# lcicek/Critic-VAE

Measured on AMD Instinct MI355X. Metric: VAE train-step images/sec on 64x64x3 frames, higher is better.
Workload: dtype f32

## Files before the change

### critic-vae_amd/csrc/common.h

```cpp
#pragma once
#include <hip/hip_runtime.h>
#include <stdint.h>
#include <stddef.h>
#include <atomic>

typedef float f32x16 __attribute__((ext_vector_type(16)));
typedef float f32x4 __attribute__((ext_vector_type(4)));
typedef __bf16 bf16x8 __attribute__((ext_vector_type(8)));

typedef __bf16 bf16x4 __attribute__((ext_vector_type(4)));

template <typename AT> struct Act;
template <> struct Act<float> {
    static constexpr bool BF16 = false;
    static __device__ __forceinline__ float ld(const float* p, size_t i) { return p[i]; }
    static __device__ __forceinline__ void st(float* p, size_t i, float v) { p[i] = v; }
    static __device__ __forceinline__ f32x4 ld4(const float* p, size_t i) { return *reinterpret_cast<const f32x4*>(p + i); }
    static __device__ __forceinline__ void st4(float* p, size_t i, f32x4 v) { *reinterpret_cast<f32x4*>(p + i) = v; }
    template <int V> using Vec = float __attribute__((ext_vector_type(V)));
    template <int V> static __device__ __forceinline__ Vec<V> ldv(const float* p, size_t i) {
        static_assert(V == 1 || V == 4, "fp32 storage: scalar or float4 accesses");
        return *reinterpret_cast<const Vec<V>*>(p + i);
    }
    template <int V> static __device__ __forceinline__ void stv(float* p, size_t i, Vec<V> v) {
// ... 63 lines not shown
    static constexpr int TILES_PER_IMG = tile_geom(H).TILES_PER_IMG;
    static_assert(TW * TH * IMGS == 128, "tile must hold 128 pixels");
};

__host__ __device__ inline int cdiv(int a, int b) { return (a + b - 1) / b; }

__device__ __forceinline__ void vm_drained() { __builtin_amdgcn_s_waitcnt(0x0F70); }

__device__ __forceinline__ int xcd_tile(int x, int G) { return (G & 7) ? x : (x & 7) * (G >> 3) + (x >> 3); }
inline int64_t align_up(int64_t v, int64_t a) { return (v + a - 1) / a * a; }

__device__ __forceinline__ float wave_sum(float v) {
#pragma unroll
    for (int o = 32; o > 0; o >>= 1) v += __shfl_xor(v, o, 64);
    return v;
}
__device__ __forceinline__ double wave_sum_d(double v) {
#pragma unroll
    for (int o = 32; o > 0; o >>= 1) v += __shfl_xor(v, o, 64);
    return v;
}

__device__ __forceinline__ bool wg_arrive_last(unsigned* counter, unsigned total, unsigned* lds_word) {
    asm volatile("s_waitcnt vmcnt(0)" ::: "memory");
    __syncthreads();
    if (threadIdx.x == 0) {
        __builtin_amdgcn_fence(__ATOMIC_RELEASE, "agent");
        asm volatile("s_waitcnt vmcnt(0)" ::: "memory");
        const unsigned t = __hip_atomic_fetch_add(counter, 1u, __ATOMIC_RELAXED, __HIP_MEMORY_SCOPE_AGENT);
        const bool last = t == total - 1;
        if (last) {
            __hip_atomic_store(counter, 0u, __ATOMIC_RELAXED, __HIP_MEMORY_SCOPE_AGENT);
            __builtin_amdgcn_fence(__ATOMIC_ACQUIRE, "agent");
            asm volatile("s_waitcnt vmcnt(0)" ::: "memory");
        }
        *lds_word = last ? 1u : 0u;
    }
    __syncthreads();
    return *lds_word != 0u;
}

void cvae_probe_begin(hipStream_t st);
void cvae_probe_end(hipStream_t st);

void cvae_set_error(const char* fmt, ...);
#define CVAE_CHECK_LAUNCH()                                                        \
    do {                                                                           \
        hipError_t e_ = hipGetLastError();                                         \
        if (e_ != hipSuccess) {                                                    \
            cvae_set_error("%s:%d launch failed: %s", __FILE__, __LINE__,          \
                           hipGetErrorString(e_));                                 \
            return (int)e_;                                                        \
        }                                                                          \
    } while (0)

struct DeviceOnce { std::atomic<uint64_t> mask{0}; };
inline int cvae_grant_lds(DeviceOnce& once, const void* kernel, int bytes) {
    int dev = 0;
    hipError_t e = hipGetDevice(&dev);
    const uint64_t bit = 1ull << (dev & 63);
    if (e == hipSuccess && (once.mask.load(std::memory_order_acquire) & bit)) return 0;
    if (e == hipSuccess) e = hipFuncSetAttribute(kernel, hipFuncAttributeMaxDynamicSharedMemorySize, bytes);
    if (e != hipSuccess) { cvae_set_error("dynamic LDS opt-in (%d bytes) failed: %s", bytes, hipGetErrorString(e)); return (int)e; }
    once.mask.fetch_or(bit, std::memory_order_release);
    return 0;
}

int cvae_num_cus();
int persistent_grid(int wgs_per_cu, int num_items);

enum ConvFamily { CONV_PER_TILE = 0, CONV_PS = 1, CONV_BIG = 2, E1_PACKED_FRAME = 1 };
struct ConvRoute {
    ConvFamily family;
    int tilesPerPartial;
};
ConvRoute conv_route(int precision, int layer, int width, bool dgrad, int64_t B);

int launch_conv_fwd(int layer, int width, int B, const float* in, const float* w, const float* bias,
                    float* out, float* bnpart, float* ws, hipStream_t st);
int64_t conv_fwd_ws_floats(int layer, int width, int B);
int launch_conv_dgrad(int layer, int width, int B, const float* dout, const float* w,
                      const float* mask_src, float* din, float* ws, hipStream_t st);
int64_t conv_dgrad_ws_floats(int layer, int width, int B);
bool conv_bf16_supported(int layer, int width);
int64_t conv_bf16_pack_floats(int ns);
int launch_pack_w_bf16(const float* const w[4], float* packed, int ns, hipStream_t st);
int launch_conv_fwd_bf16(int layer, int width, int ns, int B, const float* in, const float* packed, const float* bias, float* out,
                         float* bnpart, float* ws, hipStream_t st, int* tilesPerPartial = nullptr);
int launch_conv_dgrad_bf16(int layer, int width, int ns, int B, const float* dout, const float* packed, float* din, float* ws, hipStream_t st);
int launch_pack_up_bf16(const float* const wc[3], float* packed, int ns, hipStream_t st);
int launch_conv_up_fwd_bf16(int layer, int width, int ns, int B, const float* in, const float* packed, const float* bias, float* out, hipStream_t st);
int launch_conv_up_dgrad_bf16(int layer, int width, int ns, int B, const float* dout, const float* packed, const float* aux, float* din, hipStream_t st);
int64_t wgrad_bf16_ws_floats(int layer, int width, int B);
int launch_conv_wgrad_bf16(int layer, int width, int B, const float* in, const float* dout, float* dw, float* dbias, float* ws, hipStream_t st);
bool conv_wgrad_split_supported(int products);
int64_t wgrad_split_ws_floats(int layer, int width, int B);
int launch_conv_wgrad_split(int layer, int width, int products, int B, const float* in, const float* dout, float* dw, float* dbias,
                            float* ws, hipStream_t st);
int launch_splitk_bias_relu(const float* slab, const float* bias, float* out, int64_t slice, int KS, int C, hipStream_t st, bool out_bf16 = false);
int64_t wgrad_ws_floats(int layer, int width, int B);
int launch_conv_wgrad(int layer, int width, int B, const float* in, const float* dout, float* dw,
                      float* dbias, float* ws, hipStream_t st);
int launch_reduce_slabs(const float* slab, float* dst, int64_t n, int S, int64_t stride, hipStream_t st,
                        float* mid = nullptr, bool out_bf16 = false);
int launch_colsum(const float* src, int64_t rows, int C, float* dst, float* ws, hipStream_t st);
int64_t colsum_ws_floats(int64_t rows, int C);
static constexpr int CS_BLOCKS = 128;
__device__ __forceinline__ void colsum_stage1_block(const float* __restrict__ src, int64_t rows, int C, float* __restrict__ part,
                                                    int blk, int nblk, float* red) {
    const int c = threadIdx.x % C, rl = threadIdx.x / C, RL = 256 / C;
    const int64_t per = (rows + nblk - 1) / nblk;
    const int64_t r0 = blk * per;
    int64_t r1 = r0 + per; if (r1 > rows) r1 = rows;
    float acc = 0.f;
    for (int64_t r = r0 + rl; r < r1; r += RL) acc += src[r * C + c];
    red[threadIdx.x] = acc;
    __syncthreads();
    if (rl == 0) {
        for (int k = 1; k < RL; ++k) acc += red[k * C + c];
        part[(size_t)blk * C + c] = acc;
    }
}
int64_t col_reduce_ws_floats(int W);
int launch_col_reduce_partial(const float* in, int R, int W, int64_t stride, float* ws, hipStream_t st,
                              const float** rows_out, int* R_out, int64_t* stride_out);
int launch_col_reduce(const float* in, int R, int W, int64_t stride, float* out, float* ws, hipStream_t st, int skip_col0 = -1);
int launch_e1_fwd(int width, int B, const float* x, const float* w, const float* bias, float* y,
                  float* bnpart, hipStream_t st, bool bf16 = false, int pass = 0, const float* coef = nullptr, float* a1 = nullptr,
                  float* xp = nullptr);
int launch_e1_wgrad(int width, int B, const float* x, const float* dy, float* dw, float* dbias, float* ws,
                    hipStream_t st, bool bf16 = false, const float* const* fuse = nullptr,
                    const float* xp = nullptr);
const float* bn_bwd_bcoef(int layer, int width, int B, const float* ws);
int64_t e1_wgrad_ws_floats(int width, int B);
int launch_d4_fwd(int width, int B, const float* in, const float* w, const float* bias, float* recon,
                  hipStream_t st, bool bf16io = false);
int64_t d4_bwd_ws_floats(int width, int B);
int launch_d4_bwd(int width, int B, const float* o3, const float* d_recon, const float* recon,
                  const float* w, float* dout, float* d_o3, float* dw, float* db, float* ws,
                  hipStream_t st, bool bf16io = false);
int64_t conv_up_wc_floats(int layer);
int launch_collapse_w(int layer, const float* w, float* wc, hipStream_t st);
int launch_collapse_w3(const float* const w[3], float* const wc[3], hipStream_t st);
int64_t conv_up_ws_floats(int layer, int width, int B);
int launch_conv_up_fwd(int layer, int width, int B, const float* in, const float* wc, const float* bias,
                       float* out, float* ws, hipStream_t st);
int launch_conv_up_dgrad(int layer, int width, int B, const float* dout, const float* wc, const float* aux,
                         float* din, float* ws, hipStream_t st);
int64_t conv_up_wgrad_ws_floats(int layer, int width, int B);
int launch_conv_up_wgrad(int layer, int width, int B, const float* in, const float* dout, float* dw,
                         float* dbias, float* ws, hipStream_t st, bool bf16 = false);
int launch_up_wgrad_bf16_main(int layer, int width, int B, const float* in, const float* dout, float* slab, int Smax, int* S_out, hipStream_t st,
                              int* plan = nullptr);
int conv_wgrad_bf16_plan(int layer, int width, int B, int plan[3]);
int conv_up_wgrad_bf16_plan(int layer, int width, int B, int plan[3]);
int bn_num_tiles(int layer, int width, int B);
int launch_bn_fwd_finalize(int layer, int width, int B, const float* bnpart, const float* gamma,
                           const float* beta, float* run_mean, float* run_var, float* coef,
                           float* ws, int train, hipStream_t st, int tilesPerPartial = 1);
int launch_bn_fwd_record(int layer, int width, int B, const float* bnpart, float* ws, hipStream_t st, int tilesPerPartial,
                         double* rec, double* count);
int launch_bn_fwd_finish(int layer, int width, const double* rec, const double* count, const float* gamma, const float* beta,
                         float* run_mean, float* run_var, float* coef, hipStream_t st);
int64_t bn_fwd_ws_floats(int layer, int width);
int launch_bn_pool_act_fwd(int layer, int width, int B, const float* y, const float* coef, float* a,
                           hipStream_t st, bool bf16io = false);
// ... 119 lines not shown
```

### critic-vae_amd/csrc/conv_mfma_ps.hip

```cpp
#include "common.h"
#include "conv_epilogue.h"

struct ConvPsArgs {
    const float* in;
    const float* w;
    const float* bias;
    float* out;
    float* bnpart;
    int B;
};

typedef unsigned u32x4p __attribute__((ext_vector_type(4)));
__device__ __forceinline__ __amdgpu_buffer_rsrc_t make_rsrc_f(const void* p, unsigned bytes) {
    return __builtin_amdgcn_make_buffer_rsrc(const_cast<void*>(p), 0, (int)bytes, 0x00020000);
}
static constexpr unsigned OOBF = 0x80000000u;

template <int NT> struct KChunkPs { static constexpr int KC = NT == 32 ? 32 : 16, KCP = KC + 1; };

template <int KCH, int NCH, int H, bool DGRAD, int NT, int EPI>
__global__ __launch_bounds__(256) __attribute__((amdgpu_waves_per_eu(2, 2))) void conv5x5_mfma_ps_kernel(ConvPsArgs a, int numTiles) {
    using T = Tile<H>;
    constexpr int NB = NT / 32, NY = NCH / NT;
    constexpr int KC = KChunkPs<NT>::KC, KCP = KChunkPs<NT>::KCP, QPP = KC / 4, NCHUNK = KCH / KC;
// ... 154 lines not shown
                }
            }
    };

    if constexpr (HAS_BIAS) { for (int c = tid; c < NCH; c += 256) lds_bias[c] = a.bias[c]; }
    Item cur = setup(tile, n0), pd = cur;
    bool have_pd = false;
    load_w(cur, 0, 0);
    load_input(cur, 0);
    __syncthreads();
    int itemNo = 0;
    for (;;) {
        if (((itemNo++ ^ (blockIdx.x >= (unsigned)(G / 2))) & 1) != 0) __builtin_amdgcn_s_setprio(1); else __builtin_amdgcn_s_setprio(0);
        int itn = it + G, tilen, n0n;
        decode(itn, tilen, n0n);
        const bool have_next = itn < numItems && tilen < numTiles;
        const Item nxt = have_next ? setup(tilen, n0n) : cur;
#pragma unroll
        for (int nb = 0; nb < NB; ++nb)
#pragma unroll
            for (int g = 0; g < 4; ++g) {
                const f32x4 b4 = HAS_BIAS ? *reinterpret_cast<const f32x4*>(lds_bias + cur.n0 + nb * 32 + 8 * g + 4 * lh) : f32x4{0.f, 0.f, 0.f, 0.f};
#pragma unroll
                for (int e = 0; e < 4; ++e) acc[nb][4 * g + e] = b4[e];
            }
#pragma unroll
        for (int r = 0; r < 5; ++r) {
            __syncthreads();
            if (r == 0) store_input();
            store_w();
            if (r == 0) { if (NCHUNK > 1) load_input(cur, 1); else load_input(nxt, 0); }
            if (r < 4) load_w(cur, 0, r + 1); else if (NCHUNK > 1) load_w(cur, 1, 0); else load_w(nxt, 0, 0);
            __builtin_amdgcn_sched_barrier(0);
            if (r == 0) drain_store(pd, have_pd, 0, 0);
            if (r == 1) { drain_store(pd, have_pd, 0, 2); bn_rows(pd, 0); }
            if (r == 2 && NB > 1) { drain_store(pd, have_pd, NB - 1, 0); bn_rows(pd, NB - 1); }
            if (r == 3 && NB > 1) drain_store(pd, have_pd, NB - 1, 2);
            if (r == 4) bn_combine(pd, have_pd);
            __syncthreads();
            mfma_phase(r);
        }
        for (int cc = 1; cc < NCHUNK; ++cc) {
            const bool lastc = cc == NCHUNK - 1;
#pragma unroll
            for (int r = 0; r < 5; ++r) {
                __syncthreads();
                if (r == 0) store_input();
                store_w();
                if (r == 0) { if (lastc) load_input(nxt, 0); else load_input(cur, cc + 1); }
                if (r < 4) load_w(cur, cc, r + 1); else if (lastc) load_w(nxt, 0, 0); else load_w(cur, cc + 1, 0);
                __syncthreads();
                mfma_phase(r);
            }
        }
#pragma unroll
        for (int nb = 0; nb < NB; ++nb)
#pragma unroll
            for (int v = 0; v < 16; ++v) pend[nb][v] = RELU ? fmaxf(acc[nb][v], 0.f) : acc[nb][v];
        pd = cur; have_pd = true;
        if (!have_next) break;
        cur = nxt; it = itn;
    }
#pragma unroll
    for (int nb = 0; nb < NB; ++nb) { drain_store(pd, true, nb, 0); drain_store(pd, true, nb, 2); bn_rows(pd, nb); }
    __syncthreads();
    bn_combine(pd, true);
}

template <int KCH, int NCH, int H, bool DGRAD, int NT, int EPI>
static int run_mfma_ps(const ConvPsArgs& a, hipStream_t st) {
    using T = Tile<H>;
    constexpr int NY = NCH / NT;
    const int numTiles = cdiv(a.B, T::IMGS) * T::TILES_PER_IMG;
    const int G = persistent_grid(2, cdiv(numTiles, 8) * 8 * NY);
    cvae_probe_begin(st);
    hipLaunchKernelGGL((conv5x5_mfma_ps_kernel<KCH, NCH, H, DGRAD, NT, EPI>), dim3(G), dim3(256), 0, st, a, numTiles);
    cvae_probe_end(st);
    CVAE_CHECK_LAUNCH();
    return 0;
}

int launch_conv_mfma_ps(int layer, int width, bool dgrad, int B, const float* in, const float* w, const float* bias, float* out, float* bnpart, hipStream_t st) {
    const ConvPsArgs a{in, w, bias, out, bnpart, B};
    if (!dgrad) {
        if (width == 64) {
            switch (layer) {
                case 1: return run_mfma_ps<32, 64, 32, false, 64, EPI_BIAS_BNSTAT>(a, st);
                case 2: return run_mfma_ps<64, 128, 16, false, 64, EPI_BIAS_BNSTAT>(a, st);
                case 3: return run_mfma_ps<128, 256, 8, false, 64, EPI_BIAS_BNSTAT>(a, st);
            }
        } else if (width == 128) {
            switch (layer) {
                case 1: return run_mfma_ps<32, 64, 64, false, 64, EPI_BIAS_BNSTAT>(a, st);
                case 2: return run_mfma_ps<64, 128, 32, false, 64, EPI_BIAS_BNSTAT>(a, st);
            }
        }
    } else {
        if (width == 64) {
            switch (layer) {
                case 2: return run_mfma_ps<128, 64, 16, true, 64, EPI_PLAIN>(a, st);
                case 3: return run_mfma_ps<256, 128, 8, true, 64, EPI_PLAIN>(a, st);
            }
        } else if (width == 128) {
            switch (layer) {
                case 2: return run_mfma_ps<128, 64, 32, true, 64, EPI_PLAIN>(a, st);
            }
        }
    }
    cvae_set_error("conv_mfma_ps: no instantiation for layer %d %s at width %d", layer, dgrad ? "dgrad" : "fwd", width);
    return -2;
}
```

### critic-vae_amd/lib.py

```python
import ctypes as C
import os
import subprocess

import torch

_HERE = os.path.dirname(os.path.abspath(__file__))
LIB_PATH = os.environ.get("CVAE_LIB") or os.path.join(_HERE, "libcvae_hip.so")
N_SCALARS = 16
SYNC_DOUBLES = 2412
SYNC_POINTS = 9
SCORE_COLS = 8
SCORE_STATE_DOUBLES = 24


class CvaeError(RuntimeError):
    pass


class _Config(C.Structure):
    _fields_ = [("width", C.c_int32), ("max_batch", C.c_int32),
                ("overlap_wgrad", C.c_int32), ("precision", C.c_int32)]


class CrfParams(C.Structure):
# ... 35 lines not shown

TRACE_MAX_SCALARS = 16
TRACE_MAX_TENSORS = 32


class TraceRow(C.Structure):
    _fields_ = [("step", C.c_int64), ("lr", C.c_float), ("applied", C.c_int32), ("nonfinite", C.c_uint32),
                ("grad_norm", C.c_float), ("coef", C.c_float), ("n_scalars", C.c_int32), ("reserved", C.c_uint8 * 32),
                ("scalars", C.c_float * TRACE_MAX_SCALARS)]


class TensorStat(C.Structure):
    _fields_ = [("g2", C.c_double), ("p2", C.c_double), ("u2", C.c_double), ("gmax", C.c_float), ("pmax", C.c_float),
                ("g_nonfinite", C.c_uint32), ("p_nonfinite", C.c_uint32), ("step", C.c_int64)]


def _range_arrays(ranges):
    ranges = [(int(b), int(e)) for b, e in ranges]
    n = len(ranges)
    return n, (C.c_int64 * max(n, 1))(*[b for b, _ in ranges]), (C.c_int64 * max(n, 1))(*[e for _, e in ranges])


def tensor_stats_plan(ranges):
    lib = load()
    n, b, e = _range_arrays(ranges)
    chunk, items, grid = C.c_int32(), C.c_int32(), C.c_int32()
    if lib.cvae_tensor_stats_plan(n, b, e, C.byref(chunk), C.byref(items), C.byref(grid)) != 0:
        raise CvaeError(f"cvae_tensor_stats_plan: {lib.cvae_last_error().decode()}")
    return {"chunk": chunk.value, "items": items.value, "grid": grid.value}


def tensor_stats_scratch_bytes(ranges):
    lib = load()
    n, b, e = _range_arrays(ranges)
    size = lib.cvae_tensor_stats_scratch_bytes(n, b, e)
    if size < 0:
        raise CvaeError(f"cvae_tensor_stats_scratch_bytes: {lib.cvae_last_error().decode()}")
    return size


class AugmentParams(C.Structure):
    _fields_ = [("key", C.c_uint64), ("flip_below", C.c_uint32), ("max_shift", C.c_int32), ("gain_q16", C.c_int32),
                ("reserved", C.c_int32)]


class Panel(C.Structure):
    _fields_ = [("kind", C.c_int32), ("reserved", C.c_int32), ("data", C.c_void_p), ("batch_stride", C.c_int64)]


PANEL_F32_CHW, PANEL_U8_HWC, PANEL_U8_GREY, PANEL_MASK = 0, 1, 2, 3
MAX_PANELS = 8
COMPOSE_CLAMP = 1
CRITIC_KEEP, CRITIC_DECISIONS, CRITIC_TRAIN_FLOATS = 800, 11072, 11876
CRITIC_LOSS = {"bce": 0, "mse": 1}
CRITIC_SCORE_COLS = 8
CRITIC_SCORE_STATE_DOUBLES = 40


def build(verbose=False):
    r = subprocess.run(["make", "-j8", "-C", os.path.join(_HERE, "csrc")],
                       capture_output=not verbose, text=True)
    if r.returncode != 0:
        raise CvaeError("building libcvae_hip.so failed:\n" + (r.stdout or "") + (r.stderr or ""))
    return LIB_PATH


_lib = None
_p, _i32, _i64, _f = C.c_void_p, C.c_int32, C.c_int64, C.c_float

_SIGS = {
    "cvae_version": (C.c_char_p, []),
    "cvae_last_error": (C.c_char_p, []),
    "cvae_create": (C.c_int, [C.POINTER(_Config), C.POINTER(_p)]),
    "cvae_destroy": (None, [_p]),
    "cvae_param_total": (_i64, [_p]),
    "cvae_param_count": (_i32, [_p]),
    "cvae_param_name": (C.c_char_p, [_p, _i32]),
    "cvae_param_offset": (_i64, [_p, _i32]),
    "cvae_param_numel": (_i64, [_p, _i32]),
    "cvae_workspace_bytes": (_i64, [_p, _i32]),
    "cvae_bn_state_floats": (_i64, [_p]),
    "cvae_ws_offset": (_i64, [_p, _i32, C.c_char_p]),
    "cvae_conv_route": (_i32, [_i32, _i32, _i32, _i32, _i64]),
    "cvae_forward": (C.c_int, [_p, _i32] + [_p] * 9 + [_i32, _p]),
    "cvae_decode": (C.c_int, [_p, _i32] + [_p] * 5),
    "cvae_loss": (C.c_int, [_p, _i32] + [_p] * 10),
    "cvae_loss_obj": (C.c_int, [_p, _i32] + [_p] * 5 + [C.POINTER(Objective)] + [_p] * 5),
    "cvae_backward": (C.c_int, [_p, _i32] + [_p] * 12),
    "cvae_backward_phases": (C.c_int, [_p, _i32] + [_p] * 11 + [_i32, _p]),
    "cvae_grad_bucket": (C.c_int, [_p, _i32, C.POINTER(C.c_int64), C.POINTER(C.c_int64)]),
    "cvae_sync_slot": (C.c_int, [_i32, C.POINTER(C.c_int64), C.POINTER(C.c_int64)]),
    "cvae_forward_stage": (C.c_int, [_p, _i32] + [_p] * 9 + [_i32, _p, _i32, _p]),
    "cvae_loss_stage": (C.c_int, [_p, _i32] + [_p] * 10 + [_i32, _p]),
    "cvae_backward_stage": (C.c_int, [_p, _i32] + [_p] * 12 + [_i32, _p]),
    "cvae_scale_loss_grads": (C.c_int, [_p, _i32] + [_p] * 8),
    "cvae_adam_step": (C.c_int, [_p, _p, _p, _p, _p, _i64, _i32, _f, _f, _f, _f, _f, _p]),
    "cvae_score_cols": (_i32, []),
    "cvae_score_state_bytes": (_i64, []),
    "cvae_score_init": (C.c_int, [_p, _p, _p]),
    "cvae_score": (C.c_int, [_p, _i32] + [_p] * 8),
    "cvae_score_finish": (C.c_int, [_p, _i32, _p, _p, _p]),
    "cvae_guard_state_bytes": (_i64, []),
    "cvae_guard_init": (C.c_int, [_p, _p, _i64, _i64, _p]),
    "cvae_grad_stats": (C.c_int, [_p, _p, _i64, _f, _f, _i32, _f, _f, _f, _p, _p]),
    "cvae_adam_step_guarded": (C.c_int, [_p, _p, _p, _p, _p, _i64, _f, _p, _p]),
    "cvae_adam_step_opt": (C.c_int, [_p, _p, _p, _p, _p, _i64, _i32, _f, _f, _f, _f, _f, C.POINTER(OptArgs), _p, _p, _p, _i32, _p]),
    "cvae_adam_step_guarded_opt": (C.c_int, [_p, _p, _p, _p, _p, _i64, _f, _p, C.POINTER(OptArgs), _p, _p, _p, _i32, _p]),
    "cvae_trace_push": (C.c_int, [_p, _p, _i64, _i64, _f, _p, _i32, _p, _p]),
    "cvae_tensor_stats": (C.c_int, [_p, _p, _p, _p, _p, _i64, _i32, C.POINTER(C.c_int64), C.POINTER(C.c_int64), _i64, _f, _f, _f, _f, _f,
                                    _p, _p, _p, _p]),
    "cvae_tensor_stats_scratch_bytes": (_i64, [_i32, C.POINTER(C.c_int64), C.POINTER(C.c_int64)]),
    "cvae_tensor_stats_plan": (C.c_int, [_i32, C.POINTER(C.c_int64), C.POINTER(C.c_int64)] + [C.POINTER(C.c_int32)] * 3),
    "cvae_grads_to_bf16": (C.c_int, [_p, _p, _p, _i64, _p]),
    "cvae_grads_from_bf16": (C.c_int, [_p, _p, _p, _i64, _p]),
    "cvae_critic_param_count": (_i32, []),
    "cvae_critic_forward": (C.c_int, [_p, _i32, _p, _p, _p, _p]),
    "cvae_critic_train_floats": (_i64, []),
    "cvae_critic_grad_scratch_bytes": (_i64, [_p, _i32]),
    "cvae_critic_grad": (C.c_int, [_p, _i32, _p, _p, _p, _f, _i32] + [_p] * 7),
    "cvae_critic_score_state_bytes": (_i64, []),
    "cvae_critic_score_scratch_bytes": (_i64, [_p, _i32]),
    "cvae_critic_score_init": (C.c_int, [_p, _p, _p]),
    "cvae_critic_score": (C.c_int, [_p, _i32, _p, _p, _i64] + [_p] * 6),
    "cvae_preprocess_u8": (C.c_int, [_p, _i32, _p, _p, _p]),
    "cvae_diff_grey": (C.c_int, [_p, _i32, _p, _p, _p, _p]),
    "cvae_curate_select": (C.c_int, [_p, _i32, _p, _i64, _p, _i32, _i64] + [_p] * 6),
    "cvae_gather_frames_u8": (C.c_int, [_p, _i32, _p, _p, _i64, _p, _i64, _p, _p, _p, _i64, _p]),
    "cvae_preprocess_u8_gather": (C.c_int, [_p, _i32, _i32, _p, _p, _i64, _p, _p, _p, _p]),
    "cvae_curate_select_recon": (C.c_int, [_p, _i32, _p, _i64, _p, _i32, _i64] + [_p] * 10),
    "cvae_recon_zcat": (C.c_int, [_p, _i32, _p, _p, _p, _p, _i64, _p, _p]),
    "cvae_gather_f32": (C.c_int, [_p, _i32, _i32, _p, _p, _i64, _p, _p, _p, _p]),
    "cvae_preprocess_u8_gather_aug": (C.c_int, [_p, _i32, _i32, _p, _p, _i64, _p, C.POINTER(AugmentParams), _p, _p, _p, _p]),
    "cvae_gather_f32_aug": (C.c_int, [_p, _i32, _i32, _p, _p, _i64, _p, C.POINTER(AugmentParams), _p, _p, _p, _p]),
    "cvae_diff_normalize": (C.c_int, [_p, _i32, _p, C.c_double, C.c_double, _i32] + [_p] * 6),
    "cvae_mask_counts": (C.c_int, [_p, _i32, _p, _p, _p, _p]),
    "cvae_crf_scratch_bytes": (_i64, [_p, _i32]),
    "cvae_dense_crf": (C.c_int, [_p, _i32, _p, _p, C.POINTER(CrfParams), _p, _p, _p, _p]),
    "cvae_compose_frames": (C.c_int, [_p, _i32, _i32, C.POINTER(Panel), _i32, _i32, _p, _p, _i32, _i32, _i32, _p, _i32, _i32, _p, _p]),
    "cvae_inject_zcat": (C.c_int, [_p, _i32, _i32, _p, _p, _p, _p]),
    "cvae_probe_config": (C.c_int, [_p, C.c_uint32]),
    "cvae_probe_read": (C.c_int, [_p, _i32, C.POINTER(C.c_float), _i32]),
    "cvae_op_scratch_floats": (_i64, [_p, _i32]),
    "cvae_op_bn_partial_floats": (_i64, [_p, _i32, _i32]),
    "cvae_op_msssim_ws_floats": (_i64, [_p, _i32]),
    "cvae_op_conv_fwd": (C.c_int, [_p, _i32, _i32] + [_p] * 7),
    "cvae_op_conv_dgrad": (C.c_int, [_p, _i32, _i32] + [_p] * 6),
    "cvae_op_conv_wgrad": (C.c_int, [_p, _i32, _i32] + [_p] * 6),
    "cvae_op_d4_bwd": (C.c_int, [_p, _i32] + [_p] * 10),
    "cvae_op_bn_pool_act_fwd": (C.c_int, [_p, _i32, _i32] + [_p] * 9 + [_i32, _p]),
    "cvae_op_bn_pool_act_bwd": (C.c_int, [_p, _i32, _i32] + [_p] * 11),
    "cvae_op_conv_tiles_per_partial": (_i32, [_p, _i32, _i32]),
    "cvae_op_conv_wgrad_plan": (C.c_int, [_p, _i32, _i32, C.POINTER(C.c_int32)]),
    "cvae_op_bn_fwd_finalize": (C.c_int, [_p, _i32, _i32, _p, _i32] + [_p] * 6 + [_i32, _p]),
    "cvae_op_msssim": (C.c_int, [_p, _i32] + [_p] * 6),
    "cvae_op_latent_scratch_floats": (_i64, [_p, _i32]),
    "cvae_op_latent_plan": (_i32, [_i32, _i32, _i32, C.POINTER(C.c_int32)]),
    "cvae_op_fc_fwd": (C.c_int, [_p, _i32] + [_p] * 10),
    "cvae_op_decin_fwd": (C.c_int, [_p, _i32] + [_p] * 5),
    "cvae_op_decin_bwd": (C.c_int, [_p, _i32] + [_p] * 8),
    "cvae_op_fc_bwd": (C.c_int, [_p, _i32] + [_p] * 12),
}
EXPORTS = tuple(_SIGS)


def load():
    global _lib
# ... 549 lines not shown
```

### include/cvae.h

```cpp
#ifndef CVAE_H
#define CVAE_H

#include <stddef.h>
#include <stdint.h>

#ifdef __cplusplus
extern "C" {
#endif

typedef struct cvae_handle_s* cvae_handle;

typedef struct cvae_config {
    int32_t width;
    int32_t max_batch;
    int32_t overlap_wgrad;
    int32_t precision;
} cvae_config;

enum { CVAE_OK = 0, CVAE_EINVAL = -1, CVAE_EUNSUPPORTED = -2, CVAE_ENOWS = -3 };

#define CVAE_N_SCALARS 16

const char* cvae_version(void);
const char* cvae_last_error(void);
// ... 167 lines not shown
int cvae_preprocess_u8(cvae_handle h, int32_t batch, const uint8_t* frames_hwc, float* x, void* stream);


int cvae_curate_select(cvae_handle h, int32_t n_traj, const int64_t* traj_offsets, int64_t n_frames,
                       const float* preds, int32_t collect, int64_t total_images, int64_t* running,
                       int64_t* counts, int64_t* first, int64_t* span, int64_t* sel, void* stream);

int cvae_gather_frames_u8(cvae_handle h, int32_t width, const uint8_t* src_frames, const float* src_preds_or_null,
                          int64_t n_src, const int64_t* sel, int64_t max_count, const int64_t* span,
                          uint8_t* dst_frames, float* dst_preds_or_null, int64_t capacity, void* stream);

int cvae_preprocess_u8_gather(cvae_handle h, int32_t batch, int32_t width, const uint8_t* frames_hwc,
                              const float* preds, int64_t n_frames, const int64_t* idx, float* x,
                              float* pred, void* stream);


int cvae_curate_select_recon(cvae_handle h, int32_t n_traj, const int64_t* traj_offsets, int64_t n_frames,
                             const float* preds, int32_t collect, int64_t total_images, int64_t* running,
                             int64_t* counts, int64_t* first, int64_t* sel_first, int64_t* span, int64_t* ent_frame,
                             int32_t* ent_kind, int64_t* ent_sel, int64_t* sel, void* stream);

int cvae_recon_zcat(cvae_handle h, int32_t n_entries, const int64_t* ent_sel, const int32_t* ent_kind, const float* mu,
                    const float* sel_preds, int64_t n_sel, float* zcat, void* stream);

int cvae_gather_f32(cvae_handle h, int32_t batch, int32_t width, const float* frames, const float* preds,
                    int64_t n_frames, const int64_t* idx, float* x, float* pred, void* stream);

typedef struct cvae_augment {
    uint64_t key;
    uint32_t flip_below;
    int32_t  max_shift;
    int32_t  gain_q16;
    int32_t  reserved;
} cvae_augment;
int cvae_preprocess_u8_gather_aug(cvae_handle h, int32_t batch, int32_t width, const uint8_t* frames_hwc,
                                  const float* preds, int64_t n_frames, const int64_t* idx, const cvae_augment* aug,
                                  float* x, float* pred, int32_t* applied_or_null, void* stream);
int cvae_gather_f32_aug(cvae_handle h, int32_t batch, int32_t width, const float* frames, const float* preds,
                        int64_t n_frames, const int64_t* idx, const cvae_augment* aug, float* x, float* pred,
                        int32_t* applied_or_null, void* stream);

int cvae_diff_grey(cvae_handle h, int32_t batch, const float* recon_one, const float* recon_zero,
                   float* diff, void* stream);


int cvae_diff_normalize(cvae_handle h, int32_t batch, const float* diff, double mean_max, double diff_factor,
                        int32_t thr, const uint8_t* gt_or_null, uint8_t* diff_u8, uint8_t* mask_or_null,
                        int64_t* frame_counts_or_null, int64_t* hist_or_null, void* stream);

int cvae_mask_counts(cvae_handle h, int32_t batch, const uint8_t* mask, const uint8_t* gt,
                     int64_t* frame_counts, void* stream);

typedef struct cvae_crf_params {
    float w1, alpha, beta, w2, gamma, p_floor;
    int32_t iterations;
} cvae_crf_params;
int64_t cvae_crf_scratch_bytes(cvae_handle h, int32_t batch);
int cvae_dense_crf(cvae_handle h, int32_t batch, const uint8_t* frames_hwc, const float* prob1,
                   const cvae_crf_params* params, uint8_t* labels, float* q1_or_null, void* scratch,
                   void* stream);


enum { CVAE_PANEL_F32_CHW = 0, CVAE_PANEL_U8_HWC = 1, CVAE_PANEL_U8_GREY = 2, CVAE_PANEL_MASK = 3 };
#define CVAE_MAX_PANELS 8
#define CVAE_COMPOSE_CLAMP 1
typedef struct cvae_panel {
    int32_t kind;
    int32_t reserved;
    const void* data;
    int64_t batch_stride;
} cvae_panel;

int cvae_compose_frames(cvae_handle h, int32_t batch, int32_t n_panels, const cvae_panel* panels, int32_t row_offset,
                        int32_t flags, const uint8_t* overlay_or_null, const uint8_t* atlas_or_null, int32_t n_labels,
                        int32_t label_h, int32_t label_w, const int32_t* label_idx, int32_t label_x, int32_t label_y,
                        uint8_t* out, void* stream);

int cvae_inject_zcat(cvae_handle h, int32_t n_images, int32_t n_rewards, const float* mu, const float* rewards,
                     float* zcat, void* stream);

int64_t cvae_ws_offset(cvae_handle h, int32_t batch, const char* name);

int32_t cvae_conv_route(int32_t precision, int32_t width, int32_t layer, int32_t dgrad, int64_t batch);

int cvae_probe_config(cvae_handle h, uint32_t mask);
int cvae_probe_read(cvae_handle h, int32_t id, float* ms_host, int32_t cap);

int64_t cvae_op_scratch_floats(cvae_handle h, int32_t batch);
int64_t cvae_op_bn_partial_floats(cvae_handle h, int32_t layer, int32_t batch);
int64_t cvae_op_msssim_ws_floats(cvae_handle h, int32_t batch);

int cvae_op_conv_fwd(cvae_handle h, int32_t layer, int32_t batch, const float* in, const float* w,
                     const float* bias, float* out, float* bn_partials, void* scratch, void* stream);
int cvae_op_conv_dgrad(cvae_handle h, int32_t layer, int32_t batch, const float* dout,
                       const float* w, const float* mask_src, float* din, void* scratch, void* stream);
int cvae_op_conv_wgrad(cvae_handle h, int32_t layer, int32_t batch, const float* in,
                       const float* dout, float* dw, float* dbias, void* scratch, void* stream);
int cvae_op_d4_bwd(cvae_handle h, int32_t batch, const float* o3, const float* d_recon,
                   const float* recon, const float* w, float* dout, float* d_o3, float* dw,
                   float* db, void* scratch, void* stream);
int cvae_op_bn_pool_act_fwd(cvae_handle h, int32_t layer, int32_t batch, const float* y,
                            const float* bn_partials, const float* gamma, const float* beta,
                            float* run_mean, float* run_var, float* coef, float* a, void* scratch,
                            int32_t train, void* stream);
int32_t cvae_op_conv_tiles_per_partial(cvae_handle h, int32_t layer, int32_t batch);
int cvae_op_conv_wgrad_plan(cvae_handle h, int32_t layer, int32_t batch, int32_t* out);
int cvae_op_bn_fwd_finalize(cvae_handle h, int32_t layer, int32_t batch, const float* bn_partials,
                            int32_t tiles_per_partial, const float* gamma, const float* beta,
                            float* run_mean, float* run_var, float* coef, void* scratch,
                            int32_t train, void* stream);
int cvae_op_bn_pool_act_bwd(cvae_handle h, int32_t layer, int32_t batch, const float* y,
                            const float* a, const float* da, const float* coef, const float* gamma,
                            float* dy, float* dgamma, float* dbeta, float* dbias, void* scratch,
                            void* stream);
int cvae_op_msssim(cvae_handle h, int32_t batch, const float* img1, const float* img2, void* ws,
                   float* scalars, float* d_img1, void* stream);

int64_t cvae_op_latent_scratch_floats(cvae_handle h, int32_t batch);
#define CVAE_LATENT_PLAN_INTS 15
int32_t cvae_op_latent_plan(int32_t width, int32_t batch, int32_t num_cus, int32_t* out);
int cvae_op_fc_fwd(cvae_handle h, int32_t batch, const float* flat, const float* wfc, const float* bfc,
                   const float* eps, const float* pred, float* mu, float* logvar, float* zcat,
                   void* scratch, void* stream);
int cvae_op_decin_fwd(cvae_handle h, int32_t batch, const float* zcat, const float* wd, const float* bd,
                      float* h_out, void* stream);
int cvae_op_decin_bwd(cvae_handle h, int32_t batch, const float* zcat, const float* dh, const float* wd,
                      float* dwd, float* dbd, float* dzcat, void* scratch, void* stream);
int cvae_op_fc_bwd(cvae_handle h, int32_t batch, const float* flat, const float* wfc, const float* dzcat,
                   const float* eps, const float* logvar, const float* dmu_loss, const float* dlv_loss,
                   float* dwfc, float* dbfc, float* dflat, void* scratch, void* stream);

#ifdef __cplusplus
}
#endif
#endif
```

Before: 90190.

## Add row-structured 5x5 conv kernel for 8x8 layer 3 forward

Adds a new fp32 MFMA conv kernel for the 8x8 encoder layer-3 forward that treats each output row separately and skips the (output row, kernel row) pairs that fall entirely in zero padding. That leaves 34 of the 40 pairs. It also restructures the pipeline: a group of 8 images per item, per-kernel-row weight staging, and a double-buffered prefetch of the next item's input. The intent is to cut wasted MFMA work on padding and improve data reuse at this small spatial size. The cost is a separate code path to maintain, and it could lose to the existing tuned kernel if the extra barriers or LDS traffic dominate.

```diff
diff --git a/critic-vae_amd/csrc/common.h b/critic-vae_amd/csrc/common.h
--- a/critic-vae_amd/csrc/common.h
+++ b/critic-vae_amd/csrc/common.h
@@ -169,6 +169,7 @@
 int launch_conv_dgrad(int layer, int width, int B, const float* dout, const float* w,
                       const float* mask_src, float* din, float* ws, hipStream_t st);
 int64_t conv_dgrad_ws_floats(int layer, int width, int B);
+int launch_conv_rows_e4(int B, const float* in, const float* w, const float* bias, float* out, float* bnpart, hipStream_t st);
 bool conv_bf16_supported(int layer, int width);
 int64_t conv_bf16_pack_floats(int ns);
 int launch_pack_w_bf16(const float* const w[4], float* packed, int ns, hipStream_t st);
diff --git a/critic-vae_amd/csrc/conv_mfma_ps.hip b/critic-vae_amd/csrc/conv_mfma_ps.hip
--- a/critic-vae_amd/csrc/conv_mfma_ps.hip
+++ b/critic-vae_amd/csrc/conv_mfma_ps.hip
@@ -260,12 +260,12 @@
 
 int launch_conv_mfma_ps(int layer, int width, bool dgrad, int B, const float* in, const float* w, const float* bias, float* out, float* bnpart, hipStream_t st) {
     const ConvPsArgs a{in, w, bias, out, bnpart, B};
+    if (layer == 3 && width == 64 && !dgrad) return launch_conv_rows_e4(B, in, w, bias, out, bnpart, st);
     if (!dgrad) {
         if (width == 64) {
             switch (layer) {
                 case 1: return run_mfma_ps<32, 64, 32, false, 64, EPI_BIAS_BNSTAT>(a, st);
                 case 2: return run_mfma_ps<64, 128, 16, false, 64, EPI_BIAS_BNSTAT>(a, st);
-                case 3: return run_mfma_ps<128, 256, 8, false, 64, EPI_BIAS_BNSTAT>(a, st);
             }
         } else if (width == 128) {
             switch (layer) {
diff --git a/critic-vae_amd/csrc/conv_rows.hip b/critic-vae_amd/csrc/conv_rows.hip
--- /dev/null
+++ b/critic-vae_amd/csrc/conv_rows.hip
@@ -0,0 +1,276 @@
+#include "common.h"
+#include "conv_epilogue.h"
+
+namespace rows {
+constexpr int H = 8;
+__host__ __device__ constexpr int row_first(int y) { return y < 2 ? 2 - y : 0; }
+__host__ __device__ constexpr int row_last(int y) { return y > H - 3 ? H + 1 - y : 4; }
+__host__ __device__ constexpr bool row_runs(int y, int r) { return r >= row_first(y) && r <= row_last(y); }
+constexpr bool row_table_is_brute_force() {
+    for (int y = 0; y < H; ++y)
+        for (int r = 0; r < 5; ++r)
+            if (row_runs(y, r) != (y + r - 2 >= 0 && y + r - 2 < H)) return false;
+    return true;
+}
+constexpr int row_run_count() {
+    int n = 0;
+    for (int y = 0; y < H; ++y)
+        for (int r = 0; r < 5; ++r) n += row_runs(y, r) ? 1 : 0;
+    return n;
+}
+static_assert(row_table_is_brute_force(), "row table: (y, r) runs exactly when 0 <= y + r - 2 < 8");
+static_assert(row_run_count() == 34, "34 of the 40 (output row, kernel row) pairs run");
+
+constexpr int KC = 16;
+constexpr int CB = 16;
+constexpr int GI = 8;
+constexpr int RW = H + 4;
+constexpr int IS = H * RW + 8;
+constexpr int PS = GI * IS + 16;
+constexpr int IN_FLOATS = KC * PS, W_FLOATS = 5 * KC * CB;
+static_assert(IS % 32 == 8 && PS % 32 == 16, "fragment reads: banks x + 8 img + 16 k");
+static_assert((KC - 1) * PS + (GI - 1) * IS + (H - 1) * RW + (H - 1) + 4 < IN_FLOATS, "last fragment element inside the planes");
+}
+
+struct ConvRowsArgs {
+    const float* in;
+    const float* w;
+    const float* bias;
+    float* out;
+    float* bnpart;
+    int B;
+};
+
+typedef unsigned u32x4r __attribute__((ext_vector_type(4)));
+static constexpr unsigned OOBR = 0x80000000u;
+__device__ __forceinline__ __amdgpu_buffer_rsrc_t rows_rsrc(const void* p, unsigned bytes) {
+    return __builtin_amdgcn_make_buffer_rsrc(const_cast<void*>(p), 0, (int)bytes, 0x00020000);
+}
+__device__ __forceinline__ float oct_sum(float x) {
+    x += dpp_mov<0x141>(x);
+    x += dpp_mov<0x4E>(x);
+    x += dpp_mov<0xB1>(x);
+    return x;
+}
+
+template <int KCH, int NCH, int EPI>
+__global__ __launch_bounds__(256) __attribute__((amdgpu_waves_per_eu(2, 2))) void conv5x5_rows_kernel(ConvRowsArgs a, int numTiles) {
+    using namespace rows;
+    constexpr int NY = NCH / CB, NCHUNK = KCH / KC;
+    constexpr bool HAS_BIAS = EPI != EPI_PLAIN, BNSTAT = EPI == EPI_BIAS_BNSTAT, RELU = EPI == EPI_BIAS_RELU;
+    static_assert(KCH % KC == 0 && NCH % CB == 0, "channel tiling");
+    __shared__ __attribute__((aligned(16))) float smem[IN_FLOATS + W_FLOATS + NCH];
+    float* lds_in = smem;
+    float* lds_w = smem + IN_FLOATS;
+    float* lds_bias = lds_w + W_FLOATS;
+
+    const int tid = threadIdx.x, lane = tid & 63, wave = tid >> 6, lj = lane & 15, kq = lane >> 4;
+    const int G = gridDim.x;
+    const int numGroups = cdiv(numTiles, GI / 2), PP = cdiv(numGroups, 8), numItems = 8 * PP * NY;
+    auto decode = [&](int it, int& grp, int& n0) { const int x = it & 7, j = it >> 3, jp = j / NY; n0 = (j - jp * NY) * CB; grp = jp < PP ? x * PP + jp : numGroups; };
+    int it = blockIdx.x, grp, n0;
+    decode(it, grp, n0);
+    if (it >= numItems || grp >= numGroups) return;
+
+    const int pimg = wave * 2 + (lj >> 3), px = lj & 7;
+    const int aBase = kq * PS + pimg * IS + px;
+    const int bBase = kq * CB + lj;
+    constexpr int WQ = W_FLOATS / 4, WPT = (WQ + 255) / 256;
+    unsigned wbase[WPT];
+#pragma unroll
+    for (int i = 0; i < WPT; ++i) {
+        const int q = tid + i * 256, tap = q >> 6;
+        unsigned o = OOBR;
+        if (q < WQ) {
+            const int c4 = q & 3, kc = (q >> 2) & 15;
+            o = (unsigned)((tap * KCH + kc) * NCH + c4 * 4) * 4u;
+        }
+        wbase[i] = o;
+    }
+    constexpr int IPT = GI;
+    static_assert(H * H * (KC / 4) == 256, "input units: a thread owns one (pixel, channel quad) of every image");
+    const int sc4 = tid & 3, spix = tid >> 2;
+    const unsigned irel = (unsigned)(spix * KCH + sc4 * 4) * 4u;
+    const int sdst = sc4 * 4 * PS + (spix >> 3) * RW + (spix & 7) + 2;
+    const __amdgpu_buffer_rsrc_t rs_out = rows_rsrc(a.out, (unsigned)((size_t)a.B * H * H * NCH * 4));
+    const __amdgpu_buffer_rsrc_t rs_bn = rows_rsrc(a.bnpart, BNSTAT ? (unsigned)((size_t)2 * numTiles * NCH * 4) : 0u);
+    const __amdgpu_buffer_rsrc_t rs_w = rows_rsrc(a.w, (unsigned)(25u * KCH * NCH * 4u));
+    const __amdgpu_buffer_rsrc_t rs_in = rows_rsrc(a.in, (unsigned)((size_t)a.B * H * H * KCH * 4));
+
+    struct Item { int n0, img0; };
+    f32x4 wreg[WPT], ireg[IPT];
+    unsigned okmask = 0u;
+    auto load_w = [&](const Item& x, int cc, int r) {
+        const unsigned soff = (unsigned)((r * 5 * KCH + cc * KC) * NCH + x.n0) * 4u;
+#pragma unroll
+        for (int i = 0; i < WPT; ++i) wreg[i] = __builtin_bit_cast(f32x4, __builtin_amdgcn_raw_buffer_load_b128(rs_w, wbase[i], soff, 0));
+    };
+    auto store_w = [&]() {
+#pragma unroll
+        for (int i = 0; i < WPT; ++i) {
+            const int q = tid + i * 256;
+            if (q < WQ) *reinterpret_cast<f32x4*>(lds_w + q * 4) = wreg[i];
+        }
+    };
+    auto load_input = [&](const Item& x, int cc) {
+#pragma unroll
+        for (int i = 0; i < IPT; ++i) {
+            const unsigned okb = (unsigned)(x.img0 + i < a.B);
+            const unsigned e = okb ? (unsigned)(x.img0 * H * H * KCH * 4) + irel + (unsigned)(i * H * H * KCH * 4 + cc * KC * 4) : OOBR;
+            ireg[i] = __builtin_bit_cast(f32x4, __builtin_amdgcn_raw_buffer_load_b128(rs_in, e, 0, 0));
+            okmask = (okmask & ~(1u << i)) | (okb << i);
+        }
+    };
+    auto store_input = [&]() {
+#pragma unroll
+        for (int i = 0; i < IPT; ++i) {
+            const bool ok = (okmask >> i) & 1u;
+            float* d = lds_in + sdst + i * IS;
+            d[0] = ok ? ireg[i].x : 0.f; d[PS] = ok ? ireg[i].y : 0.f; d[2 * PS] = ok ? ireg[i].z : 0.f; d[3 * PS] = ok ? ireg[i].w : 0.f;
+        }
+    };
+
+    f32x4 acc[H], pend[H];
+#pragma unroll
+    for (int y = 0; y < H; ++y) pend[y] = f32x4{0.f, 0.f, 0.f, 0.f};
+
+    auto drain_store = [&](const Item& pd, bool have_pd) {
+        const bool ok = have_pd && pd.img0 + pimg < a.B;
+        const unsigned base = ((unsigned)((pd.img0 + pimg) * H * H + px) * NCH + pd.n0 + 4 * kq) * 4u;
+#pragma unroll
+        for (int y = 0; y < H; ++y)
+            __builtin_amdgcn_raw_buffer_store_b128(__builtin_bit_cast(u32x4r, pend[y]), rs_out, ok ? base + (unsigned)(y * H * NCH * 4) : OOBR, 0, 0);
+    };
+    auto bn_partial = [&](const Item& pd, bool have_pd) {
+        if constexpr (BNSTAT) {
+            const bool valid = pd.img0 + pimg < a.B;
+            f32x4 S, M;
+#pragma unroll
+            for (int v = 0; v < 4; ++v) {
+                float sw[2], qw[2];
+#pragma unroll
+                for (int h = 0; h < 2; ++h) {
+                    float t[4], u[4];
+#pragma unroll
+                    for (int yy = 0; yy < 4; ++yy) { t[yy] = valid ? pend[4 * h + yy][v] : 0.f; u[yy] = t[yy] * t[yy]; asm volatile("" : "+v"(u[yy])); }
+                    sw[h] = oct_sum((t[0] + t[2]) + (t[1] + t[3]));
+                    qw[h] = oct_sum((u[0] + u[2]) + (u[1] + u[3]));
+                }
+                const bool hi = lj >= 8;
+                const float so0 = dpp_mov<0x128>(sw[0]), so1 = dpp_mov<0x128>(sw[1]), qo0 = dpp_mov<0x128>(qw[0]), qo1 = dpp_mov<0x128>(qw[1]);
+                float s = 0.f, q = 0.f;
+                s += hi ? so0 : sw[0]; s += hi ? so1 : sw[1]; s += hi ? sw[0] : so0; s += hi ? sw[1] : so1;
+                q += hi ? qo0 : qw[0]; q += hi ? qo1 : qw[1]; q += hi ? qw[0] : qo0; q += hi ? qw[1] : qo1;
+                int nvalid_img = a.B - (pd.img0 + wave * 2);
+                if (nvalid_img > 2) nvalid_img = 2;
+                if (nvalid_img < 1) nvalid_img = 1;
+                const double cnt = (double)(nvalid_img * H * H);
+                const double m2 = (double)q - (double)s * (double)s / cnt;
+                S[v] = s; M[v] = (float)(m2 > 0.0 ? m2 : 0.0);
+            }
+            const int mt = pd.img0 / 2 + wave;
+            const bool ok = have_pd && lj == 0 && mt < numTiles;
+            const unsigned o = (unsigned)(mt * NCH + pd.n0 + 4 * kq) * 4u;
+            __builtin_amdgcn_raw_buffer_store_b128(__builtin_bit_cast(u32x4r, S), rs_bn, ok ? o : OOBR, 0, 0);
+            __builtin_amdgcn_raw_buffer_store_b128(__builtin_bit_cast(u32x4r, M), rs_bn, ok ? o + (unsigned)(numTiles * NCH) * 4u : OOBR, 0, 0);
+        }
+    };
+    auto mfma_phase = [&](int r) {
+        const float* ap = lds_in + aBase;
+        const float* wp = lds_w + bBase;
+#pragma unroll
+        for (int s = 0; s < 5; ++s)
+#pragma unroll
+            for (int g = 0; g < KC / 4; ++g) {
+                const float wv = wp[(s * KC + g * 4) * CB];
+#pragma unroll
+                for (int y = 0; y < H; ++y)
+                    if (row_runs(y, r)) acc[y] = __builtin_amdgcn_mfma_f32_16x16x4f32(wv, ap[g * 4 * PS + (y + r - 2) * RW + s], acc[y], 0, 0, 0);
+            }
+    };
+
+    for (int i = tid; i < IN_FLOATS; i += 256) lds_in[i] = 0.f;
+    if constexpr (HAS_BIAS) { for (int c = tid; c < NCH; c += 256) lds_bias[c] = a.bias[c]; }
+    Item cur{n0, grp * GI}, pd = cur;
+    bool have_pd = false;
+    load_w(cur, 0, 0);
+    load_input(cur, 0);
+    __syncthreads();
+    int itemNo = 0;
+    for (;;) {
+        if (((itemNo++ ^ (blockIdx.x >= (unsigned)(G / 2))) & 1) != 0) __builtin_amdgcn_s_setprio(1); else __builtin_amdgcn_s_setprio(0);
+        int itn = it + G, grpn, n0n;
+        decode(itn, grpn, n0n);
+        const bool have_next = itn < numItems && grpn < numGroups;
+        const Item nxt = have_next ? Item{n0n, grpn * GI} : cur;
+        {
+            const f32x4 b4 = HAS_BIAS ? *reinterpret_cast<const f32x4*>(lds_bias + cur.n0 + 4 * kq) : f32x4{0.f, 0.f, 0.f, 0.f};
+#pragma unroll
+            for (int y = 0; y < H; ++y) acc[y] = b4;
+        }
+#pragma unroll
+        for (int r = 0; r < 5; ++r) {
+            __syncthreads();
+            if (r == 0) store_input();
+            store_w();
+            if (r == 0) { if (NCHUNK > 1) load_input(cur, 1); else load_input(nxt, 0); }
+            if (r < 4) load_w(cur, 0, r + 1); else if (NCHUNK > 1) load_w(cur, 1, 0); else load_w(nxt, 0, 0);
+            if (r == 0) {
+                __builtin_amdgcn_sched_barrier(0);
+                drain_store(pd, have_pd);
+                bn_partial(pd, have_pd);
+            }
+            __syncthreads();
+            mfma_phase(r);
+        }
+        for (int cc = 1; cc < NCHUNK; ++cc) {
+            const bool lastc = cc == NCHUNK - 1;
+#pragma unroll
+            for (int r = 0; r < 5; ++r) {
+                __syncthreads();
+                if (r == 0) store_input();
+                store_w();
+                if (r == 0) { if (lastc) load_input(nxt, 0); else load_input(cur, cc + 1); }
+                if (r < 4) load_w(cur, cc, r + 1); else if (lastc) load_w(nxt, 0, 0); else load_w(cur, cc + 1, 0);
+                __syncthreads();
+                mfma_phase(r);
+            }
+        }
+#pragma unroll
+        for (int y = 0; y < H; ++y)
+#pragma unroll
+            for (int v = 0; v < 4; ++v) pend[y][v] = RELU ? fmaxf(acc[y][v], 0.f) : acc[y][v];
+        pd = cur; have_pd = true;
+        if (!have_next) break;
+        cur = nxt; it = itn;
+    }
+    drain_store(pd, true);
+    bn_partial(pd, true);
+}
+
+template <int KCH, int NCH, int EPI>
+static int run_rows(const ConvRowsArgs& a, hipStream_t st) {
+    const int numTiles = cdiv(a.B, 2);
+    const int G = persistent_grid(2, cdiv(cdiv(numTiles, rows::GI / 2), 8) * 8 * (NCH / rows::CB));
+    cvae_probe_begin(st);
+    hipLaunchKernelGGL((conv5x5_rows_kernel<KCH, NCH, EPI>), dim3(G), dim3(256), 0, st, a, numTiles);
+    cvae_probe_end(st);
+    CVAE_CHECK_LAUNCH();
+    return 0;
+}
+
+extern "C" int32_t cvae_conv_rows_table(int32_t* runs) {
+    int32_t n = 0;
+    for (int y = 0; y < rows::H; ++y)
+        for (int r = 0; r < 5; ++r) {
+            const int32_t on = rows::row_runs(y, r) ? 1 : 0;
+            if (runs) runs[y * 5 + r] = on;
+            n += on;
+        }
+    return n;
+}
+
+int launch_conv_rows_e4(int B, const float* in, const float* w, const float* bias, float* out, float* bnpart, hipStream_t st) {
+    const ConvRowsArgs a{in, w, bias, out, bnpart, B};
+    return run_rows<128, 256, EPI_BIAS_BNSTAT>(a, st);
+}
diff --git a/critic-vae_amd/lib.py b/critic-vae_amd/lib.py
--- a/critic-vae_amd/lib.py
+++ b/critic-vae_amd/lib.py
@@ -141,6 +141,7 @@
     "cvae_bn_state_floats": (_i64, [_p]),
     "cvae_ws_offset": (_i64, [_p, _i32, C.c_char_p]),
     "cvae_conv_route": (_i32, [_i32, _i32, _i32, _i32, _i64]),
+    "cvae_conv_rows_table": (_i32, [_p]),
     "cvae_forward": (C.c_int, [_p, _i32] + [_p] * 9 + [_i32, _p]),
     "cvae_decode": (C.c_int, [_p, _i32] + [_p] * 5),
     "cvae_loss": (C.c_int, [_p, _i32] + [_p] * 10),
diff --git a/include/cvae.h b/include/cvae.h
--- a/include/cvae.h
+++ b/include/cvae.h
@@ -273,6 +273,8 @@
 int64_t cvae_ws_offset(cvae_handle h, int32_t batch, const char* name);
 
 int32_t cvae_conv_route(int32_t precision, int32_t width, int32_t layer, int32_t dgrad, int64_t batch);
+
+int32_t cvae_conv_rows_table(int32_t* runs);
 
 int cvae_probe_config(cvae_handle h, uint32_t mask);
 int cvae_probe_read(cvae_handle h, int32_t id, float* ms_host, int32_t cap);
```

After: 90130. No clear change (-0.1%).
